# researchmm/MM-Diffusion

Hardware: AMD Instinct MI355X
Metric: denoising steps/sec (video+audio pair), 16x64x64 / 25600 (higher is better)
Workload: dtype bf16; 1 GPU; BASELINE configs[1]: Landscape base model (133.68M params), DDPM p_sample, timestep_respacing=250, per-GPU batch 4, 16x3x64x64 video + 1x25600 audio; global_batch=4, parallelism=batch-sharded x1, no in-loop collective, weights=key-seeded synthetic (mm_diffusion.synth), graph_replay=True, batch_lanes=2, finite=True, ranks_seen=1

## Files before the change

### mm-diffusion_amd/build.py

```python
#!/usr/bin/env python3
import os
import subprocess
import sys

HERE = os.path.dirname(os.path.abspath(__file__))
SRC = os.path.join(HERE, "csrc")
OUT = os.path.join(HERE, "lib", "libmmd.so")
SOURCES = ["mmd_core.hip", "mmd_gemm.hip", "mmd_vconv.hip", "mmd_tattn.hip", "mmd_tconv.hip", "mmd_aconv.hip", "mmd_norm.hip", "mmd_attn.hip", "mmd_misc.hip", "mmd_bwd.hip", "mmd_attn_bwd.hip", "mmd_attn_bwd_mfma.hip"]
FLAGS = ["--offload-arch=gfx950", "-O3", "-std=c++17", "-fPIC", "-ffp-contract=fast", "-Wno-unused-result", "-Wno-inline-asm"]
FLAGS += os.environ.get("MMD_EXTRA_CXXFLAGS", "").split()
NO_PACKED_F32 = ["-Xclang", "-target-feature", "-Xclang", "-packed-fp32-ops"]
FLAGS += NO_PACKED_F32


def _stale():
    if not os.path.exists(OUT):
        return True
    t = os.path.getmtime(OUT)
    deps = [os.path.join(SRC, f) for f in os.listdir(SRC)] + [os.path.abspath(__file__)]
    return any(os.path.getmtime(d) > t for d in deps)


def _llvm_bin():
    cands = [os.environ.get("LLVM_BIN")]
    hipcc = os.environ.get("HIPCC", "/opt/rocm/bin/hipcc")
    try:
        out = subprocess.run([hipcc, "--print-prog-name=llvm-objdump"], stdout=subprocess.PIPE, stderr=subprocess.DEVNULL, timeout=60).stdout.decode().strip()
        if out and os.path.isabs(out):
            cands.append(os.path.dirname(out))
    except (OSError, subprocess.SubprocessError):
        pass
    cands += [os.path.join(os.path.dirname(os.path.dirname(os.path.realpath(hipcc))), "lib", "llvm", "bin"), "/opt/rocm/lib/llvm/bin"]
    for d in cands:
        if d and os.path.exists(os.path.join(d, "llvm-objdump")):
            return d
    raise RuntimeError("build check: llvm-objdump not found (looked in %s); set LLVM_BIN to the LLVM bin directory of the ROCm toolchain"
                       % ", ".join(str(d) for d in cands if d))


def _check_no_packed_f32(path):
    import re
    import tempfile
    llvm = _llvm_bin()
    with tempfile.TemporaryDirectory() as td:
        lib = os.path.join(td, "lib.so")
        os.symlink(os.path.abspath(path), lib)
        subprocess.check_call([os.path.join(llvm, "llvm-objdump"), "--offloading", lib], cwd=td, stdout=subprocess.DEVNULL, stderr=subprocess.DEVNULL)
        cos = sorted(f for f in os.listdir(td) if f.endswith("gfx950"))
        if len(cos) < len(SOURCES) - 1:
            raise RuntimeError("build check: expected >= %d gfx950 code objects in %s, found %d" % (len(SOURCES) - 1, path, len(cos)))
        asm = ""
        for f in cos:
            asm += subprocess.run([os.path.join(llvm, "llvm-objdump"), "-d", "--mcpu=gfx950", os.path.join(td, f)],
                                  stdout=subprocess.PIPE, stderr=subprocess.DEVNULL, check=True).stdout.decode(errors="replace")
    n_mfma = len(re.findall(r"\bv_mfma_", asm))
    bad = re.findall(r"\bv_pk_(?:add|mul|fma)_f32\b", asm)
    if n_mfma == 0:
        raise RuntimeError("build check: the disassembly of %s shows no v_mfma instruction - the check looked at the wrong object" % path)
    if bad:
        raise RuntimeError("build check: %d packed-fp32 instruction(s) (%s ...) in %s: the device pass ignored %s" %
                           (len(bad), bad[0], path, " ".join(NO_PACKED_F32)))


def _check_strip_asm(obj):
    import importlib.util
    spec = importlib.util.spec_from_file_location("strip_asm_check", os.path.join(os.path.dirname(HERE), "tools", "strip_asm_check.py"))
    chk = importlib.util.module_from_spec(spec)
    spec.loader.exec_module(chk)
    chk.LLVM = _llvm_bin()
    n, bad = chk.check(chk.disassemble(obj))
    if n == 0 or bad:
        raise RuntimeError("build check: conv1x1_strip_res_kernel: %d kernels checked, %d violations%s" % (n, len(bad), (": " + bad[0]) if bad else ""))


def build(force=False, verbose=True):
    if not force and not _stale():
        return OUT
    os.makedirs(os.path.dirname(OUT), exist_ok=True)
    hipcc = os.environ.get("HIPCC", "/opt/rocm/bin/hipcc")
    objs = []
    procs = []
    for s in SOURCES:
        o = os.path.join(HERE, "lib", s.replace(".hip", ".o"))
        objs.append(o)
        cmd = [hipcc, *FLAGS, "-c", os.path.join(SRC, s), "-o", o]
        procs.append((cmd, subprocess.Popen(cmd, stdout=subprocess.PIPE, stderr=subprocess.STDOUT)))
    for cmd, p in procs:
        out, _ = p.communicate()
        if p.returncode != 0:
            raise RuntimeError("hipcc failed: %s\n%s" % (" ".join(cmd), out.decode()))
        lines = out.decode().splitlines()
        text = "\n".join(ln for ln in lines if "'-packed-fp32-ops' is not a recognized feature" not in ln).strip()
        if verbose and text:
            print(text)
    tmp = OUT + ".tmp"
    cmd = [hipcc, "--offload-arch=gfx950", "-shared", "-fPIC", "-o", tmp, *objs]
    try:
        subprocess.check_call(cmd)
        _check_no_packed_f32(tmp)
        _check_strip_asm(os.path.join(HERE, "lib", "mmd_gemm.o"))
        os.replace(tmp, OUT)
    finally:
        if os.path.exists(tmp):
            os.remove(tmp)
    if verbose:
        print("built", OUT)
    return OUT


if __name__ == "__main__":
    build(force="--force" in sys.argv)
```

### mm-diffusion_amd/csrc/mmd_common.h

```cpp
#pragma once
#include <hip/hip_runtime.h>
#include <stdint.h>
#include <stdio.h>
#include <stdarg.h>
#include "../../include/mmd.h"

#define MMD_F32 0
#define MMD_BF16 1

#define MMD_OK 0
#define MMD_ERR_ARG (-1)
#define MMD_ERR_LAUNCH (-2)
#define MMD_ERR_UNSUPPORTED (-3)

typedef __attribute__((ext_vector_type(8))) __bf16 bf16x8;
typedef __attribute__((ext_vector_type(4))) __bf16 bf16x4;
typedef __attribute__((ext_vector_type(16))) float f32x16;
typedef __attribute__((ext_vector_type(4))) float f32x4;
typedef __attribute__((ext_vector_type(4))) uint32_t u32x4;
typedef __attribute__((ext_vector_type(2))) uint32_t u32x2;

int mmd_set_error(int code, const char* fmt, ...);
int mmd_check_launch(const char* what);

#define MMD_REQUIRE(cond, ...)                                  \
  do {                                                          \
    if (!(cond)) return mmd_set_error(MMD_ERR_ARG, __VA_ARGS__); \
  } while (0)

__device__ __forceinline__ float bf16_bits_to_f32(uint32_t bits16) { return __uint_as_float(bits16 << 16); }
__device__ __forceinline__ uint32_t f32_to_bf16_bits(float f) {
  uint32_t u = __float_as_uint(f);
  if ((u & 0x7fffffffu) > 0x7f800000u) return 0x7fc0u;
  u += 0x7fffu + ((u >> 16) & 1u);
  return u >> 16;
}
__device__ __forceinline__ uint32_t pack_bf16x2(float lo, float hi) {
  return f32_to_bf16_bits(lo) | (f32_to_bf16_bits(hi) << 16);
}

template <typename T> struct Elt;
template <> struct Elt<float> {
  static constexpr int EPV = 4;
  static constexpr int DT = MMD_F32;
  __device__ static __forceinline__ void unpack(const u32x4& v, float* f) {
#pragma unroll
    for (int i = 0; i < 4; ++i) f[i] = __uint_as_float(v[i]);
  }
  __device__ static __forceinline__ u32x4 pack(const float* f) {
    u32x4 v;
#pragma unroll
    for (int i = 0; i < 4; ++i) v[i] = __float_as_uint(f[i]);
    return v;
  }
  __device__ static __forceinline__ float ld(const void* p, int64_t i) { return ((const float*)p)[i]; }
  __device__ static __forceinline__ void st(void* p, int64_t i, float v) { ((float*)p)[i] = v; }
};
template <> struct Elt<__bf16> {
  static constexpr int EPV = 8;
  static constexpr int DT = MMD_BF16;
  __device__ static __forceinline__ void unpack(const u32x4& v, float* f) {
#pragma unroll
    for (int i = 0; i < 4; ++i) {
      f[2 * i] = __uint_as_float(v[i] << 16);
      f[2 * i + 1] = __uint_as_float(v[i] & 0xffff0000u);
    }
  }
  __device__ static __forceinline__ u32x4 pack(const float* f) {
    bf16x8 t;
#pragma unroll
    for (int i = 0; i < 8; ++i) t[i] = (__bf16)f[i];
    return __builtin_bit_cast(u32x4, t);
  }
  __device__ static __forceinline__ float ld(const void* p, int64_t i) {
    return bf16_bits_to_f32(((const uint16_t*)p)[i]);
  }
  __device__ static __forceinline__ void st(void* p, int64_t i, float v) {
    ((__bf16*)p)[i] = (__bf16)v;
  }
};

__device__ __forceinline__ float silu_f(float x) { return x * __builtin_amdgcn_rcpf(1.0f + __expf(-x)); }

__device__ __forceinline__ float wave_sum(float v) {
#pragma unroll
  for (int o = 32; o > 0; o >>= 1) v += __shfl_xor(v, o, 64);
  return v;
}
__device__ __forceinline__ double wave_sum_d(double v) {
#pragma unroll
  for (int o = 32; o > 0; o >>= 1) v += __shfl_xor(v, o, 64);
  return v;
}
__device__ __forceinline__ float wave_max(float v) {
#pragma unroll
  for (int o = 32; o > 0; o >>= 1) v = fmaxf(v, __shfl_xor(v, o, 64));
  return v;
}

template <int CTRL, int ROWS>
__device__ __forceinline__ float dpp_add(float v) {
  return v + __builtin_bit_cast(float, __builtin_amdgcn_update_dpp(0, __builtin_bit_cast(int, v), CTRL, ROWS, 0xf, false));
}
__device__ __forceinline__ float halfwave_total(float v) {
  v = dpp_add<0x128, 0xf>(v);
  v = dpp_add<0x124, 0xf>(v);
  v = dpp_add<0x122, 0xf>(v);
  v = dpp_add<0x121, 0xf>(v);
  return dpp_add<0x142, 0xa>(v);
}


static inline int cdiv(int64_t a, int64_t b) { return (int)((a + b - 1) / b); }

#define MMD_MAX_DEVICES 16
static inline int mmd_device_slot() {
  int d = 0;
  (void)hipGetDevice(&d);
  return d & (MMD_MAX_DEVICES - 1);
}
```

### mm-diffusion_amd/csrc/mmd_gemm.hip

```cpp
#include "mmd_common.h"

struct ConvGemmParams {
  const char* A; int64_t lda;
  const char* W;
  const float* bias;
  const char* R; int64_t ldr;
  char* Y; int64_t ldy;
  int M, Cout, Cin, ntaps;
  int D0, D1, D2;
  const float* gn_a; const float* gn_b;
  int gn_act, gn_S;
  int64_t gn_rows;
  float* stats; int64_t stats_ld;
  int taps[27 * 3];
};

template <int BM, int BN>
__device__ __forceinline__ void epilogue_stats(const ConvGemmParams& p, float (&sum)[BM / 64][8], float (&sq)[BM / 64][8], float* sP, int m0,
                                               int n0, int tid) {
  constexpr int CVN = BN / 8, NREC = BM / 64;
  const int lane = tid & 63, wave = tid >> 6, cg = tid % CVN;
#pragma unroll
  for (int r = 0; r < NREC; ++r)
#pragma unroll
// ... 1744 lines not shown
  bool& attr_set = attr_done[mmd_device_slot()];
  if (!attr_set) {
    hipError_t e = hipFuncSetAttribute((const void*)conv_gemm_halo_kernel<T, GN>, hipFuncAttributeMaxDynamicSharedMemorySize, (int)lds);
    if (e != hipSuccess) return mmd_set_error(MMD_ERR_LAUNCH, "conv_gemm_halo: set LDS attr: %s", hipGetErrorString(e));
    attr_set = true;
  }
  const int grid = (p.M / 128) * cdiv(p.Cout, 128);
  hipLaunchKernelGGL((conv_gemm_halo_kernel<T, GN>), dim3(grid), dim3(256), lds, st, p);
  return mmd_check_launch("conv_gemm_halo");
}

template <bool GN>
static int launch_conv_gemm_halo16(const ConvGemmParams& p, hipStream_t st) {
  bool taps_ok = p.ntaps == 9;
  for (int t = 0; t < p.ntaps && taps_ok; ++t)
    taps_ok = p.taps[t * 3] == 0 && p.taps[t * 3 + 1] == t / 3 - 1 && p.taps[t * 3 + 2] == t % 3 - 1;
  if (!taps_ok || p.D1 % 16 != 0 || p.D2 % 16 != 0 || (int64_t)p.D0 * p.D1 * p.D2 != p.M || p.Cin % 64 != 0 ||
      ((int64_t)p.D1 * p.D2 - 1) * p.lda * 2 + (int64_t)p.Cin * 2 >= 0x7fffffffLL || (int64_t)128 * p.Cin * 9 * 2 >= 0x7fffffffLL)
    return mmd_set_error(MMD_ERR_UNSUPPORTED, "conv_gemm tile 133 (halo, 16 x 16 patches): needs the nine spatial taps in row-major (dh, dw) order, "
                         "D1 %% 16 == 0, D2 %% 16 == 0, full frames, Cin %% 64 == 0 and frames below 2 GB");
  if (GN && p.gn_rows % ((int64_t)p.D1 * p.D2) != 0)
    return mmd_set_error(MMD_ERR_UNSUPPORTED, "conv_gemm tile 133 with fused GroupNorm: needs slices of whole frames");
  constexpr size_t OPS_B = 2 * (size_t)(41 * 8 * 128) + 3 * (size_t)(128 * 128), C_B = 256 * 132 * sizeof(float);
  const size_t lds = (OPS_B > C_B ? OPS_B : C_B) + 1024 + 256;
  static bool attr_done[MMD_MAX_DEVICES] = {};
  bool& attr_set = attr_done[mmd_device_slot()];
  if (!attr_set) {
    hipError_t e = hipFuncSetAttribute((const void*)conv_gemm_halo16_kernel<GN>, hipFuncAttributeMaxDynamicSharedMemorySize, (int)lds);
    if (e != hipSuccess) return mmd_set_error(MMD_ERR_LAUNCH, "conv_gemm_halo16: set LDS attr: %s", hipGetErrorString(e));
    attr_set = true;
  }
  const int grid = (p.M / 256) * cdiv(p.Cout, 128);
  hipLaunchKernelGGL((conv_gemm_halo16_kernel<GN>), dim3(grid), dim3(512), lds, st, p);
  return mmd_check_launch("conv_gemm_halo16");
}

template <typename T>
static bool glds_desc_ok(const ConvGemmParams& p) {
  static const bool on = [] { const char* e = getenv("MMD_GEMM_DESC"); return !(e && e[0] == '0'); }();
  constexpr int ES = 16 / Elt<T>::EPV;
  int maxshift = 0;
  for (int t = 0; t < p.ntaps; ++t) {
    const int64_t sh = ((int64_t)p.taps[3 * t] * p.D1 * p.D2 + (int64_t)p.taps[3 * t + 1] * p.D2 + p.taps[3 * t + 2]) * p.lda * ES;
    if (sh > 0x3fffffff || sh < -0x3fffffff) return false;
    (void)maxshift;
  }
  return on && ((int64_t)p.M * p.lda + p.Cin) * ES < 0x7fffffffLL && (int64_t)128 * p.Cin * p.ntaps * ES < 0x7fffffffLL;
}

template <typename T>
static int launch_conv_gemm_glds(const ConvGemmParams& p, hipStream_t st) {
  const size_t lds = 128 * 132 * sizeof(float) + 336;
  static bool attr_done[MMD_MAX_DEVICES] = {};
  bool& attr_set = attr_done[mmd_device_slot()];
  if (!attr_set) {
    hipError_t e = hipFuncSetAttribute((const void*)conv_gemm_glds_kernel<T, false, 2, false>, hipFuncAttributeMaxDynamicSharedMemorySize, (int)lds);
    if (e == hipSuccess) e = hipFuncSetAttribute((const void*)conv_gemm_glds_kernel<T, true, 2, false>, hipFuncAttributeMaxDynamicSharedMemorySize, (int)lds);
    if (e == hipSuccess) e = hipFuncSetAttribute((const void*)conv_gemm_glds_kernel<T, true, 2, true>, hipFuncAttributeMaxDynamicSharedMemorySize, (int)lds);
    if (e != hipSuccess) return mmd_set_error(MMD_ERR_LAUNCH, "conv_gemm_glds: set LDS attr: %s", hipGetErrorString(e));
    attr_set = true;
  }
  const int grid = cdiv(p.M, 128) * cdiv(p.Cout, 128);
  if (p.Cin % (8 * Elt<T>::EPV) != 0) hipLaunchKernelGGL((conv_gemm_glds_kernel<T, false, 2, false>), dim3(grid), dim3(256), lds, st, p);
  else if (glds_desc_ok<T>(p)) hipLaunchKernelGGL((conv_gemm_glds_kernel<T, true, 2, true>), dim3(grid), dim3(256), lds, st, p);
  else hipLaunchKernelGGL((conv_gemm_glds_kernel<T, true, 2, false>), dim3(grid), dim3(256), lds, st, p);
  return mmd_check_launch("conv_gemm_glds");
}

template <typename T>
static int launch_conv_gemm_ring(const ConvGemmParams& p, hipStream_t st) {
  if (p.Cin % (8 * Elt<T>::EPV) != 0)
    return mmd_set_error(MMD_ERR_UNSUPPORTED, "conv_gemm tile 132 (deep ring): Cin must be a multiple of one 128-byte K step");
  const size_t lds = 8 * (size_t)(128 * 128) + 336;
  static bool attr_done[MMD_MAX_DEVICES] = {};
  bool& attr_set = attr_done[mmd_device_slot()];
  if (!attr_set) {
    hipError_t e = hipFuncSetAttribute((const void*)conv_gemm_glds_kernel<T, true, 4, false>, hipFuncAttributeMaxDynamicSharedMemorySize, (int)lds);
    if (e == hipSuccess) e = hipFuncSetAttribute((const void*)conv_gemm_glds_kernel<T, true, 4, true>, hipFuncAttributeMaxDynamicSharedMemorySize, (int)lds);
    if (e != hipSuccess) return mmd_set_error(MMD_ERR_LAUNCH, "conv_gemm_ring: set LDS attr: %s", hipGetErrorString(e));
    attr_set = true;
  }
  const int grid = cdiv(p.M, 128) * cdiv(p.Cout, 128);
  if (glds_desc_ok<T>(p)) hipLaunchKernelGGL((conv_gemm_glds_kernel<T, true, 4, true>), dim3(grid), dim3(256), lds, st, p);
  else hipLaunchKernelGGL((conv_gemm_glds_kernel<T, true, 4, false>), dim3(grid), dim3(256), lds, st, p);
  return mmd_check_launch("conv_gemm_ring");
}

template <typename T, int BM, int BN, bool GN>
static int launch_conv_gemm(const ConvGemmParams& p, hipStream_t st) {
  const size_t lds_ops = 2 * (size_t)(BM + BN) * ROWB;
  const size_t lds_c = (size_t)BM * (BN + 4) * sizeof(float);
  const size_t lds = (lds_ops > lds_c ? lds_ops : lds_c) + 336 + (GN ? 16 * 256 : 0);
  static bool attr_done[MMD_MAX_DEVICES] = {};
  bool& attr_set = attr_done[mmd_device_slot()];
  if (!attr_set) {
    hipError_t e = hipFuncSetAttribute((const void*)conv_gemm_kernel<T, BM, BN, GN>,
                                       hipFuncAttributeMaxDynamicSharedMemorySize, (int)lds);
    if (e != hipSuccess) return mmd_set_error(MMD_ERR_LAUNCH, "conv_gemm: set LDS attr: %s", hipGetErrorString(e));
    attr_set = true;
  }
  const int grid = cdiv(p.M, BM) * cdiv(p.Cout, BN);
  hipLaunchKernelGGL((conv_gemm_kernel<T, BM, BN, GN>), dim3(grid), dim3(256), lds, st, p);
  return mmd_check_launch("conv_gemm");
}

template <typename T>
static int dispatch_conv_gemm(const ConvGemmParams& p, int tile, hipStream_t st) {
  if (tile == 133) {
    if constexpr (Elt<T>::EPV == 8) return p.gn_a ? launch_conv_gemm_halo16<true>(p, st) : launch_conv_gemm_halo16<false>(p, st);
    else return mmd_set_error(MMD_ERR_UNSUPPORTED, "conv_gemm tile 133: bf16 only");
  }
  if (p.gn_a) {
    if (tile == 130) {
      if constexpr (Elt<T>::EPV == 8) return launch_conv_gemm_halo<T, true>(p, st);
      else return mmd_set_error(MMD_ERR_UNSUPPORTED, "conv_gemm tile 130 with fused GroupNorm: bf16 only");
    }
    if (tile == 128) return launch_conv_gemm<T, 128, 128, true>(p, st);
    return launch_conv_gemm<T, 64, 64, true>(p, st);
  }
  if (tile == 129) return launch_conv_gemm_glds<T>(p, st);
  if (tile == 132) return launch_conv_gemm_ring<T>(p, st);
  if (tile == 130) return launch_conv_gemm_halo<T, false>(p, st);
  if (tile == 128) return launch_conv_gemm<T, 128, 128, false>(p, st);
  return launch_conv_gemm<T, 64, 64, false>(p, st);
}

static int conv_gemm_impl(int dtype, const void* A, int64_t lda, const void* W, const float* bias, const void* R, int64_t ldr,
                          void* Y, int64_t ldy, int M, int Cout, int Cin, int ntaps, const int* taps, int D0, int D1, int D2,
                          int tile, const float* gn_a, const float* gn_b, int gn_act, int gn_S, int64_t gn_rows, float* stats,
                          int64_t stats_ld, void* stream) {
  const int epv = dtype == MMD_BF16 ? 8 : 4;
  MMD_REQUIRE(dtype == MMD_BF16 || dtype == MMD_F32, "conv_gemm: bad dtype %d", dtype);
  MMD_REQUIRE(A && W && Y && M > 0 && Cout > 0 && Cin > 0, "conv_gemm: null/empty argument");
  MMD_REQUIRE(ntaps >= 1 && ntaps <= 27 && taps, "conv_gemm: ntaps %d out of [1,27]", ntaps);
  MMD_REQUIRE(Cin % epv == 0, "conv_gemm: Cin %d must be a multiple of %d", Cin, epv);
  MMD_REQUIRE(Cout % 8 == 0, "conv_gemm: Cout %d must be a multiple of 8", Cout);
  MMD_REQUIRE(lda % epv == 0 && ldy % epv == 0 && (!R || ldr % epv == 0), "conv_gemm: row strides must be 16-byte multiples");
  MMD_REQUIRE(((uintptr_t)A | (uintptr_t)W | (uintptr_t)Y | (uintptr_t)R) % 16 == 0, "conv_gemm: pointers must be 16-byte aligned");
  MMD_REQUIRE(D0 > 0 && D1 > 0 && D2 > 0, "conv_gemm: bad position dims");
  MMD_REQUIRE(!gn_a || (gn_b && (ntaps == 1 || tile == 130 || tile == 133) && gn_S > 0 && gn_rows >= 128 && (Cin <= 256 || tile == 131 || tile == 130 || tile == 133) &&
                        (int64_t)gn_S * gn_rows == M),
              "gn_conv1x1 / gn_conv_gemm: needs contiguous slices of >= 128 rows covering M, Cin <= 256 unless tile 130 / 131, taps only with tile 130 "
              "(got S=%d rows=%ld Cin=%d M=%d ntaps=%d tile=%d)", gn_S, (long)gn_rows, Cin, M, ntaps, tile);
  ConvGemmParams p;
  p.A = (const char*)A; p.lda = lda; p.W = (const char*)W; p.bias = bias;
  p.R = (const char*)R; p.ldr = ldr; p.Y = (char*)Y; p.ldy = ldy;
  p.M = M; p.Cout = Cout; p.Cin = Cin; p.ntaps = ntaps; p.D0 = D0; p.D1 = D1; p.D2 = D2;
  p.gn_a = gn_a; p.gn_b = gn_b; p.gn_act = gn_act; p.gn_S = gn_S; p.gn_rows = gn_rows;
  MMD_REQUIRE(!stats || (M % 64 == 0 && Cout % 4 == 0 && stats_ld >= Cout / 4 && tile != 130 && tile != 133 && (uintptr_t)stats % 8 == 0),
              "conv_gemm: output statistics need M %% 64 == 0, Cout %% 4 == 0, stats_ld >= Cout / 4 (quads) and a row-tiled main loop (not tiles 130 / 133)");
  p.stats = stats; p.stats_ld = stats_ld;
  for (int i = 0; i < ntaps * 3; ++i) p.taps[i] = taps[i];
  hipStream_t st = (hipStream_t)stream;
  if (tile == 0) tile = (int64_t)cdiv(M, 128) * cdiv(Cout, 128) >= 320 ? 128 : 64;
  MMD_REQUIRE(tile == 64 || tile == 128 || ((tile == 129 || tile == 132) && !gn_a) || (tile == 130 && (!gn_a || dtype == MMD_BF16)) ||
                  ((tile == 131 || tile == 133) && dtype == MMD_BF16),
              "conv_gemm: tile must be 0, 64, 128, 129 (128 direct-to-LDS), 130 (halo-tile 3x3), 131 (row strip, bf16 1x1 convs) or 132 (129 with a "
              "four-slot ring for launches of few tiles)");
  if (tile == 131) return dispatch_conv1x1_strip(p, st);
  return dtype == MMD_BF16 ? dispatch_conv_gemm<__bf16>(p, tile, st) : dispatch_conv_gemm<float>(p, tile, st);
}

extern "C" int mmd_conv_gemm(int dtype, const void* A, int64_t lda, const void* W, const float* bias, const void* R, int64_t ldr,
                             void* Y, int64_t ldy, int M, int Cout, int Cin, int ntaps, const int* taps, int D0, int D1, int D2,
                             int tile, void* stream) {
  return conv_gemm_impl(dtype, A, lda, W, bias, R, ldr, Y, ldy, M, Cout, Cin, ntaps, taps, D0, D1, D2, tile, nullptr, nullptr, 0, 0,
                        0, nullptr, 0, stream);
}

extern "C" int mmd_conv_gemm_stats(int dtype, const void* A, int64_t lda, const void* W, const float* bias, const void* R, int64_t ldr,
                                   void* Y, int64_t ldy, int M, int Cout, int Cin, int ntaps, const int* taps, int D0, int D1, int D2,
                                   int tile, float* stats, int64_t stats_ld, void* stream) {
  MMD_REQUIRE(stats, "conv_gemm_stats: null statistics buffer");
  return conv_gemm_impl(dtype, A, lda, W, bias, R, ldr, Y, ldy, M, Cout, Cin, ntaps, taps, D0, D1, D2, tile, nullptr, nullptr, 0, 0,
                        0, stats, stats_ld, stream);
}

extern "C" int mmd_gn_conv1x1(int dtype, const void* A, int64_t lda, const float* gn_a, const float* gn_b, int act, int S,
                              int64_t rows_per_slice, const void* W, const float* bias, const void* R, int64_t ldr, void* Y,
                              int64_t ldy, int M, int Cout, int Cin, int tile, void* stream) {
  static const int tap0[3] = {0, 0, 0};
  MMD_REQUIRE(gn_a && gn_b, "gn_conv1x1: null GroupNorm affine");
  return conv_gemm_impl(dtype, A, lda, W, bias, R, ldr, Y, ldy, M, Cout, Cin, 1, tap0, 1, 1, 1, tile, gn_a, gn_b, act, S,
                        rows_per_slice, nullptr, 0, stream);
}

extern "C" int mmd_gn_conv1x1_stats(int dtype, const void* A, int64_t lda, const float* gn_a, const float* gn_b, int act, int S,
                                    int64_t rows_per_slice, const void* W, const float* bias, const void* R, int64_t ldr, void* Y,
                                    int64_t ldy, int M, int Cout, int Cin, int tile, float* stats, int64_t stats_ld, void* stream) {
  static const int tap0[3] = {0, 0, 0};
  MMD_REQUIRE(gn_a && gn_b && stats, "gn_conv1x1_stats: null GroupNorm affine / statistics buffer");
  return conv_gemm_impl(dtype, A, lda, W, bias, R, ldr, Y, ldy, M, Cout, Cin, 1, tap0, 1, 1, 1, tile, gn_a, gn_b, act, S,
                        rows_per_slice, stats, stats_ld, stream);
}

extern "C" int mmd_gn_conv_gemm(int dtype, const void* A, int64_t lda, const float* gn_a, const float* gn_b, int act, int S,
                                int64_t rows_per_slice, const void* W, const float* bias, const void* R, int64_t ldr, void* Y,
                                int64_t ldy, int M, int Cout, int Cin, int ntaps, const int* taps, int D0, int D1, int D2, int tile,
                                void* stream) {
  MMD_REQUIRE(gn_a && gn_b, "gn_conv_gemm: null GroupNorm affine");
  MMD_REQUIRE(tile == 130 || tile == 133, "gn_conv_gemm: the fused input GroupNorm of a conv with taps exists on the halo tiles (130 / 133) only");
  return conv_gemm_impl(dtype, A, lda, W, bias, R, ldr, Y, ldy, M, Cout, Cin, ntaps, taps, D0, D1, D2, tile, gn_a, gn_b, act, S,
                        rows_per_slice, nullptr, 0, stream);
}
```

### mm-diffusion_amd/mm_diffusion/ops.py

```python
import math
import os

import torch

from . import _hip as H

GN_EPS = 1e-5

_recorder = None
_keep = None


class recording:
    def __init__(self, plan, keep=None):
        self.plan, self.keep = plan, keep

    def __enter__(self):
        global _recorder, _keep
        self._prev, _recorder = (_recorder, _keep), self.plan
        _keep = self.keep
        return self.plan

    def __exit__(self, *a):
        global _recorder, _keep
# ... 165 lines not shown
        b = alloc(geom.S, C, dtype=torch.float32, device=x.device)
    if out is not None:
        _chk2d(out)
    _dispatch("mmd_gn_group", H.dt_of(x), x.data_ptr(), x.stride(0), H.ptr(out), 0 if out is None else out.stride(0), C, *geom.args(),
              gamma.data_ptr(), beta.data_ptr(), H.ptr(film), 0 if film is None else film.stride(0), GN_EPS, 1 if act else 0,
              H.ptr(a), H.ptr(b), H.ptr(mr),
              meta=(f"gn_group[S={geom.S},Tn={geom.Tn},C={C}]", 0, (1 if out is None else 2) * geom.S * geom.Tn * C * x.element_size()))
    return (a, b) if out is None else out


def add_rowbias(x, e, rows_per_sample):
    _chk2d(x)
    _dispatch("mmd_add_rowbias", H.dt_of(x), x.data_ptr(), x.stride(0), x.shape[0], x.shape[1], rows_per_sample,
           e.data_ptr(), e.stride(0))
    return x


def colsum_slices(dy, out, rows_per_sample):
    _chk2d(dy)
    S = dy.shape[0] // rows_per_sample
    _dispatch("mmd_colsum_slices", H.dt_of(dy), dy.data_ptr(), dy.stride(0), S, rows_per_sample, dy.shape[1], out.data_ptr(), out.stride(0))
    return out


TAPS_1 = [(0, 0, 0)]
TAPS_SPATIAL = [(0, dh, dw) for dh in (-1, 0, 1) for dw in (-1, 0, 1)]
TAPS_TEMPORAL = [(df, 0, 0) for df in (-1, 0, 1)]
TAPS_TEMPORAL_D1 = [(0, df, 0) for df in (-1, 0, 1)]
TAPS_3D = [(df, dh, dw) for df in (-1, 0, 1) for dh in (-1, 0, 1) for dw in (-1, 0, 1)]


def taps_audio(dilation):
    return [(-dilation, 0, 0), (0, 0, 0), (dilation, 0, 0)]


AUTOTUNE = True
_tile_cache = {}


def _pick_tile(key, launch, M, Cout, candidates=(64, 128, 129), out=None, scratch=()):
    default = (129 if 129 in candidates else 128) if ((M + 127) // 128) * ((Cout + 127) // 128) >= 320 else 64
    if default not in candidates:
        default = candidates[0]
    if not AUTOTUNE or _recorder is None:
        return default
    key = (key, tuple(candidates))
    if key in _tile_cache:
        return _tile_cache[key]
    import ctypes
    verify = out is not None and not any(t is not None and t.untyped_storage().data_ptr() == out.untyped_storage().data_ptr() for t in scratch)
    saved = []
    if verify:
        for t in scratch:
            if t is not None:
                saved.append((t, t.clone()))
                t.normal_()
    best, best_ms, ref = default, None, None
    ev = [ctypes.c_void_p(), ctypes.c_void_p()]
    for e in ev:
        H.call("mmd_event_create", ctypes.byref(e))
    st = H.stream_handle()
    for tile in candidates:
        launch(tile)
        if verify:
            if ref is None:
                ref = out.clone()
            elif tile == 130:
                err = float((out.float() - ref.float()).norm() / ref.float().norm().clamp_min(1e-30))
                if not err < (1e-2 if out.element_size() == 2 else 1e-5):
                    raise H.MMDError(f"conv_gemm tile 130 disagrees with tile {candidates[0]} on {key}: rel-L2 {err:.3e}")
            elif not torch.equal(out.view(torch.int16 if out.element_size() == 2 else torch.int32),
                                 ref.view(torch.int16 if ref.element_size() == 2 else torch.int32)):
                raise H.MMDError(f"GEMM tile {tile} is not bitwise equal to tile {candidates[0]} on {key}")
        t_min = None
        for _ in range(2):
            H.call("mmd_event_record", ev[0], st)
            for _ in range(5):
                launch(tile)
            H.call("mmd_event_record", ev[1], st)
            ms = ctypes.c_float()
            H.call("mmd_event_elapsed_ms", ev[0], ev[1], ctypes.byref(ms))
            t_min = ms.value if t_min is None else min(t_min, ms.value)
        if best_ms is None or t_min < best_ms:
            best, best_ms = tile, t_min
    for e in ev:
        H.lib().mmd_event_destroy(e)
    for t, keep in saved:
        t.copy_(keep)
    _tile_cache[key] = best
    return best


_HALO_MODE = os.environ.get("MMD_GEMM_HALO", "pin")
HALO_CANDIDATE = _HALO_MODE == "1"


def halo_tile_ok(x, taps, dims):
    M, Cin = x.shape
    return (len(taps) > 1 and all(t[0] == 0 and abs(t[1]) <= 1 and abs(t[2]) <= 1 for t in taps) and dims[1] % 8 == 0
            and dims[2] % 16 == 0 and dims[0] * dims[1] * dims[2] == M and Cin % (128 // x.element_size()) == 0)


_HALO16 = os.environ.get("MMD_HALO16", "1") != "0"


def halo_tile_code(x, taps, dims):
    return 133 if (_HALO16 and x.dtype == torch.bfloat16 and len(taps) == 9 and dims[1] % 16 == 0 and dims[2] % 16 == 0
                   and x.shape[1] >= 256 and tuple(tuple(t) for t in taps) == tuple(TAPS_SPATIAL)) else 130


def _stats_args(stats, M, Cout):
    if (stats.dtype != torch.float32 or Cout % 4 or tuple(stats.shape) != (M // 64, Cout // 4, 2) or M % 64 or stats.stride(1) != 2
            or stats.stride(2) != 1):
        raise H.MMDError(f"GEMM output statistics: expected an fp32 [M/64, Cout/4, 2] view, got {tuple(stats.shape)} strides {stats.stride()}")
    return stats.data_ptr(), stats.stride(0) // 2


_HALO_MIN_PIXELS = int(os.environ.get("MMD_HALO_MIN_PIXELS", "1024"))


def halo_tile_pinned(x, taps, dims):
    return (_HALO_MODE == "pin" and x.dtype == torch.bfloat16 and len(taps) == 9 and dims[1] * dims[2] >= _HALO_MIN_PIXELS
            and halo_tile_ok(x, taps, dims))


_STRIP_MODE = os.environ.get("MMD_GEMM_STRIP", "pin")


def strip_tile_ok(x, Cout, taps=TAPS_1, stats=None, geom=None, base=False):
    M, Cin = x.shape
    K = len(taps) * Cin
    if x.dtype != torch.bfloat16 or K not in (128, 256, 384, 512) or Cin % 64:
        return False
    if len(taps) == 1 and tuple(taps[0]) != (0, 0, 0):
        return False
    rf = 2 if K <= 256 else 1
    if Cout % (32 * rf) or Cout > 2048 or (stats is not None and M % 64):
        return False
    if base and (len(taps) != 1 or K == 512 or (stats is not None and rf != 2)):
        return False
    if geom is not None and not (len(taps) == 1 and geom.inner == 1 and geom.tstride == 1 and geom.outer_stride == geom.Tn
                                 and geom.Tn >= 128 * rf and geom.S * geom.Tn == M):
        return False
    return True


def strip_tile_pinned(x, Cout, taps=TAPS_1, stats=None, geom=None):
    if _STRIP_MODE == "0":
        return False
    return strip_tile_ok(x, Cout, taps, stats, geom, base=_STRIP_MODE == "base")


def _tile_name(tile):
    return {129: "128glds", 130: "128halo", 131: "strip", 132: "128ring", 133: "256halo"}.get(tile, tile)


_RING_MODE = os.environ.get("MMD_GEMM_RING", "1")


def ring_tile_candidate(x, Cout, ntaps):
    M, Cin = x.shape
    kstep = 128 // x.element_size()
    return (_RING_MODE != "0" and Cin % kstep == 0 and (Cin * ntaps) // kstep >= 4
            and ((M + 127) // 128) * ((Cout + 127) // 128) <= 384)


def conv_gemm(x, w, bias, taps=TAPS_1, dims=(1, 1, 1), residual=None, out=None, tile=0, stats=None):
    _chk2d(x)
    M, Cin = x.shape
    Cout = w.shape[0]
    if w.dtype != x.dtype or w.shape[1] != len(taps) * Cin or not w.is_contiguous():
        raise H.MMDError(f"conv_gemm: weight {tuple(w.shape)} {w.dtype} does not match input {tuple(x.shape)} {x.dtype} x {len(taps)} taps")
    out = alloc(M, Cout, dtype=x.dtype, device=x.device) if out is None else out
    _chk2d(out)
    arr, nt = H.taps_array(taps)
    es = x.element_size()
    base = (H.dt_of(x), x.data_ptr(), x.stride(0), w.data_ptr(), H.ptr(bias), H.ptr(residual),
            0 if residual is None else residual.stride(0), out.data_ptr(), out.stride(0), M, Cout, Cin, nt, arr,
            int(dims[0]), int(dims[1]), int(dims[2]))
    if tile == 0 and stats is None and halo_tile_pinned(x, taps, dims):
        tile = halo_tile_code(x, taps, dims)
    if tile == 0 and strip_tile_pinned(x, Cout, taps, stats):
        tile = 131
    if tile == 0:
        cands = (128, 129) if stats is not None else (64, 128, 129) + ((130,) if HALO_CANDIDATE and halo_tile_ok(x, taps, dims) else ())
        if ring_tile_candidate(x, Cout, nt):
            cands = cands + (132,)
        tile = _pick_tile((es, M, Cin, nt, Cout, residual is not None, False, tuple(dims) if 130 in cands else None),
                          lambda t: H.call("mmd_conv_gemm", *base, t, H.stream_handle()), M, Cout, cands, out=out, scratch=(x, residual))
    flops = 2 * M * Cout * Cin * nt
    nbytes = es * (M * Cin + M * Cout * (2 if residual is not None else 1) + Cout * Cin * nt) + 4 * Cout
    label = f"conv_gemm<{'bf16' if es == 2 else 'f32'},{_tile_name(tile)}>[M={M},K={Cin * nt},N={Cout}]"
    if stats is not None:
        _dispatch("mmd_conv_gemm_stats", *base, tile, *_stats_args(stats, M, Cout), meta=(label, flops, nbytes))
    else:
        _dispatch("mmd_conv_gemm", *base, tile, meta=(label, flops, nbytes))
    return out


_STRIP_BLOCKS_RULE = int(os.environ.get("MMD_STRIP_BLOCKS_RULE", "448"))


def strip_column_split(M, K, Cout):
    rf, cc = (2, 64) if K <= 256 else (1, 32)
    rowblocks, nch, n = -(-M // (128 * rf)), Cout // cc, 1
    for d in range(1, min(nch, 16) + 1):
        if nch % d == 0:
            n = d
            if rowblocks * d >= _STRIP_BLOCKS_RULE:
                break
    return n


def gn_fusable(geom: Geom, Cin, Cout, x=None, stats=None, act=False):
    if x is not None and strip_tile_pinned(x, Cout, stats=stats):
        if not strip_tile_pinned(x, Cout, stats=stats, geom=geom):
            return False
        return not (act and strip_column_split(x.shape[0], Cin, Cout) > 2)
    return (geom.inner == 1 and geom.tstride == 1 and geom.outer_stride == geom.Tn and geom.Tn >= 128 and Cin <= 256
            and (Cout + 127) // 128 <= 2)


def gn_conv1x1(x, a, b, geom: Geom, act, w, bias, residual=None, out=None, tile=0, stats=None):
    _chk2d(x)
    M, Cin = x.shape
    Cout = w.shape[0]
    if w.dtype != x.dtype or w.shape[1] != Cin or not w.is_contiguous():
        raise H.MMDError(f"gn_conv1x1: weight {tuple(w.shape)} {w.dtype} does not match input {tuple(x.shape)} {x.dtype}")
    out = alloc(M, Cout, dtype=x.dtype, device=x.device) if out is None else out
    _chk2d(out)
    es = x.element_size()
    tiled_ok = (geom.inner == 1 and geom.tstride == 1 and geom.outer_stride == geom.Tn and geom.Tn >= 128 and Cin <= 256
                and (Cout + 127) // 128 <= 2)
    strip_ok = strip_tile_ok(x, Cout, stats=stats, geom=geom)
    if not ((tile == 131 and strip_ok) or (tile in (64, 128) and tiled_ok) or (tile == 0 and (tiled_ok or strip_ok))):
        raise H.MMDError("gn_conv1x1: needs contiguous slices of >= 128 rows, Cin <= 256 (use gn_apply + conv_gemm otherwise)")
    base = (H.dt_of(x), x.data_ptr(), x.stride(0), a.data_ptr(), b.data_ptr(), 1 if act else 0, geom.S, geom.Tn,
            w.data_ptr(), H.ptr(bias), H.ptr(residual),
            0 if residual is None else residual.stride(0), out.data_ptr(), out.stride(0), M, Cout, Cin)
    if tile == 0 and strip_tile_pinned(x, Cout, stats=stats, geom=geom):
        tile = 131
    if tile == 0 and not tiled_ok:
        raise H.MMDError("gn_conv1x1: the row-strip kernel is switched off (MMD_GEMM_STRIP) and the tiled loader cannot take this launch")
    if tile == 0:
        tile = _pick_tile((es, M, Cin, 1, Cout, residual is not None, True),
                          lambda t: H.call("mmd_gn_conv1x1", *base, t, H.stream_handle()), M, Cout,
                          candidates=(128,) if stats is not None else (64, 128), out=out, scratch=(x, residual, a, b))
    nbytes = es * (M * Cin + M * Cout * (2 if residual is not None else 1) + Cout * Cin) + 4 * Cout
    meta = (f"gn_conv1x1<{'bf16' if es == 2 else 'f32'},{_tile_name(tile)}>[M={M},K={Cin},N={Cout}]", 2 * M * Cout * Cin, nbytes)
    if stats is not None:
        _dispatch("mmd_gn_conv1x1_stats", *base, tile, *_stats_args(stats, M, Cout), meta=meta)
    else:
        _dispatch("mmd_gn_conv1x1", *base, tile, meta=meta)
    return out


_HALO_GN = os.environ.get("MMD_HALO_GN", "1") != "0"


def halo_gn_ok(x, taps, dims, geom: Geom):
    return (_HALO_GN and halo_tile_pinned(x, taps, dims) and geom.inner == 1 and geom.tstride == 1 and geom.outer_stride == geom.Tn
            and geom.S * geom.Tn == x.shape[0] and geom.Tn % (dims[1] * dims[2]) == 0)


def gn_conv_gemm(x, a, b, geom: Geom, act, w, bias, taps, dims, residual=None, out=None, tile=0):
    _chk2d(x)
    M, Cin = x.shape
    Cout = w.shape[0]
    if w.dtype != x.dtype or w.shape[1] != len(taps) * Cin or not w.is_contiguous():
        raise H.MMDError(f"gn_conv_gemm: weight {tuple(w.shape)} {w.dtype} does not match input {tuple(x.shape)} {x.dtype} x {len(taps)} taps")
    if not (halo_tile_ok(x, taps, dims) and len(taps) == 9 and x.dtype == torch.bfloat16 and geom.S * geom.Tn == M
            and geom.inner == 1 and geom.tstride == 1 and geom.outer_stride == geom.Tn and geom.Tn % (dims[1] * dims[2]) == 0):
        raise H.MMDError("gn_conv_gemm: needs a bf16 3x3 conv tile 130 accepts and contiguous slices of whole frames")
    out = alloc(M, Cout, dtype=x.dtype, device=x.device) if out is None else out
    _chk2d(out)
    arr, nt = H.taps_array(taps)
    es = x.element_size()
    flops = 2 * M * Cout * Cin * nt
    nbytes = es * (M * Cin + M * Cout * (2 if residual is not None else 1) + Cout * Cin * nt) + 4 * Cout
    _dispatch("mmd_gn_conv_gemm", H.dt_of(x), x.data_ptr(), x.stride(0), a.data_ptr(), b.data_ptr(), 1 if act else 0, geom.S, geom.Tn,
              w.data_ptr(), H.ptr(bias), H.ptr(residual), 0 if residual is None else residual.stride(0), out.data_ptr(), out.stride(0),
              M, Cout, Cin, nt, arr, int(dims[0]), int(dims[1]), int(dims[2]), tile or halo_tile_code(x, taps, dims),
              meta=(f"gn_conv_gemm<bf16,{_tile_name(tile or halo_tile_code(x, taps, dims))}>[M={M},K={Cin * nt},N={Cout}]", flops, nbytes))
    return out


_VCONV_FUSED = os.environ.get("MMD_VCONV_FUSED", "1") != "0"


def vconv_shape_ok(x, Cout, N, F, Hh, Ww):
    return (x.dtype == torch.bfloat16 and F == 16 and Cout == 128 and x.shape[1] % 32 == 0 and Hh % 4 == 0 and Ww % 4 == 0
            and x.shape[0] == N * F * Hh * Ww and (16 * Hh * Ww * x.stride(0) + x.shape[1]) * 2 < 2 ** 31)


def _ranges_overlap(x, y):
    x0, y0 = x.data_ptr(), y.data_ptr()
    x1 = x0 + ((x.shape[0] - 1) * x.stride(0) + x.shape[1]) * x.element_size()
    y1 = y0 + ((y.shape[0] - 1) * y.stride(0) + y.shape[1]) * y.element_size()
    return not (x1 <= y0 or y1 <= x0)


def vconv_fused_ok(x, Cout, N, F, Hh, Ww, out=None):
    return _VCONV_FUSED and vconv_shape_ok(x, Cout, N, F, Hh, Ww) and (out is None or not _ranges_overlap(x, out))


def vconv_pack(ws, wt):
    H.require_cuda(ws, wt)
    Cout, Cin = ws.shape[0], ws.shape[1] // 9
    if ws.dtype != torch.bfloat16 or wt.dtype != torch.bfloat16 or tuple(wt.shape) != (Cout, 3 * Cout) or not ws.is_contiguous() or not wt.is_contiguous():
        raise H.MMDError(f"vconv_pack: expected contiguous bf16 [Cout, 9 Cin] / [Cout, 3 Cout], got {tuple(ws.shape)} / {tuple(wt.shape)}")
    out = torch.empty(H.lib().mmd_vconv2d1d_weight_bytes(Cin) // 2, dtype=torch.bfloat16, device=ws.device)
    H.call("mmd_vconv2d1d_pack", ws.data_ptr(), wt.data_ptr(), out.data_ptr(), Cin, Cout, H.stream_handle())
    return out


def vconv2d1d(x, wf, bias_s, bias_t, N, F, Hh, Ww, a=None, b=None, geom=None, act=True, out=None, stats=None):
    _chk2d(x)
    M, Cin = x.shape
    Cout = 128
    if not vconv_shape_ok(x, Cout, N, F, Hh, Ww):
        raise H.MMDError(f"vconv2d1d: unsupported launch (x {tuple(x.shape)} {x.dtype}, N={N} F={F} H={Hh} W={Ww})")
    if (a is None) != (b is None) or (a is not None and (geom is None or geom.inner != 1 or geom.tstride != 1 or geom.outer_stride != geom.Tn
                                                         or geom.S * geom.Tn != M or geom.Tn % (F * Hh * Ww))):
        raise H.MMDError("vconv2d1d: the fused input norm needs contiguous slices of whole samples")
    out = alloc(M, Cout, dtype=x.dtype, device=x.device) if out is None else out
    _chk2d(out)
    if _ranges_overlap(x, out) or tuple(out.shape) != (M, Cout) or out.dtype != x.dtype:
        raise H.MMDError("vconv2d1d: the output must be a bf16 [M, 128] tensor whose address range does not overlap the input's (the C side "
                         "compares whole ranges: column slices of one buffer count as overlapping)")
    if wf.numel() * wf.element_size() != H.lib().mmd_vconv2d1d_weight_bytes(Cin):
        raise H.MMDError("vconv2d1d: the weight image does not match Cin (pack it with vconv_pack)")
    sp, sld = (None, 0) if stats is None else _stats_args(stats, M, Cout)
    flops = 2 * M * Cout * (9 * Cin + 3 * Cout)
    nbytes = 2 * (M * Cin + M * Cout + Cout * (9 * Cin + 3 * Cout)) + 8 * Cout
    _dispatch("mmd_vconv2d1d", x.data_ptr(), x.stride(0), H.ptr(a), H.ptr(b), 1 if act else 0, 0 if geom is None else geom.S,
              0 if geom is None else geom.Tn, wf.data_ptr(), H.ptr(bias_s), H.ptr(bias_t), out.data_ptr(), out.stride(0), N, F, Hh, Ww, Cin, Cout,
              sp, sld, meta=(f"vconv2d1d<bf16{',gn' if a is not None else ''}>[M={M},Cin={Cin},N={Cout}]", flops, nbytes))
    return out


# ... 471 lines not shown
```

Baseline: 364.6 pair-steps/s.

## Add frame-resident 3x3 conv GEMM tile for 8x8 frames as autotune candidate

```diff
diff --git a/mm-diffusion_amd/build.py b/mm-diffusion_amd/build.py
--- a/mm-diffusion_amd/build.py
+++ b/mm-diffusion_amd/build.py
@@ -6,7 +6,7 @@
 HERE = os.path.dirname(os.path.abspath(__file__))
 SRC = os.path.join(HERE, "csrc")
 OUT = os.path.join(HERE, "lib", "libmmd.so")
-SOURCES = ["mmd_core.hip", "mmd_gemm.hip", "mmd_vconv.hip", "mmd_tattn.hip", "mmd_tconv.hip", "mmd_aconv.hip", "mmd_norm.hip", "mmd_attn.hip", "mmd_misc.hip", "mmd_bwd.hip", "mmd_attn_bwd.hip", "mmd_attn_bwd_mfma.hip"]
+SOURCES = ["mmd_core.hip", "mmd_gemm.hip", "mmd_fconv.hip", "mmd_vconv.hip", "mmd_tattn.hip", "mmd_tconv.hip", "mmd_aconv.hip", "mmd_norm.hip", "mmd_attn.hip", "mmd_misc.hip", "mmd_bwd.hip", "mmd_attn_bwd.hip", "mmd_attn_bwd_mfma.hip"]
 FLAGS = ["--offload-arch=gfx950", "-O3", "-std=c++17", "-fPIC", "-ffp-contract=fast", "-Wno-unused-result", "-Wno-inline-asm"]
 FLAGS += os.environ.get("MMD_EXTRA_CXXFLAGS", "").split()
 NO_PACKED_F32 = ["-Xclang", "-target-feature", "-Xclang", "-packed-fp32-ops"]
diff --git a/mm-diffusion_amd/csrc/mmd_common.h b/mm-diffusion_amd/csrc/mmd_common.h
--- a/mm-diffusion_amd/csrc/mmd_common.h
+++ b/mm-diffusion_amd/csrc/mmd_common.h
@@ -22,6 +22,9 @@
 
 int mmd_set_error(int code, const char* fmt, ...);
 int mmd_check_launch(const char* what);
+int mmd_fconv_dispatch(int dtype, const void* A, int64_t lda, const void* W, const float* bias, const void* R, int64_t ldr, void* Y,
+                       int64_t ldy, int M, int Cout, int Cin, int ntaps, const int* taps, int D0, int D1, int D2, bool extras,
+                       hipStream_t st);
 
 #define MMD_REQUIRE(cond, ...)                                  \
   do {                                                          \
diff --git a/mm-diffusion_amd/csrc/mmd_fconv.hip b/mm-diffusion_amd/csrc/mmd_fconv.hip
--- /dev/null
+++ b/mm-diffusion_amd/csrc/mmd_fconv.hip
@@ -0,0 +1,271 @@
+#include "mmd_common.h"
+
+struct FConvParams {
+  const char* A; int64_t lda;
+  const char* W;
+  const float* bias;
+  const char* R; int64_t ldr;
+  char* Y; int64_t ldy;
+  int M, Cout, Cin;
+};
+
+#define FCONV_FENCE() __builtin_amdgcn_sched_barrier(0)
+#define FCONV_LAUNDER4(v) asm volatile("" : "+v"((v).x), "+v"((v).y), "+v"((v).z), "+v"((v).w))
+
+__device__ __attribute__((aligned(16))) uint32_t g_fconv_zero[4] = {0, 0, 0, 0};
+
+__device__ __forceinline__ void fconv_wait_vm(int n) {
+  if (n >= 8) {
+    if (n >= 28) asm volatile("s_waitcnt vmcnt(28)" ::: "memory");
+    else if (n >= 24) asm volatile("s_waitcnt vmcnt(24)" ::: "memory");
+    else if (n >= 20) asm volatile("s_waitcnt vmcnt(20)" ::: "memory");
+    else if (n >= 16) asm volatile("s_waitcnt vmcnt(16)" ::: "memory");
+    else if (n >= 12) asm volatile("s_waitcnt vmcnt(12)" ::: "memory");
+    else if (n >= 10) asm volatile("s_waitcnt vmcnt(10)" ::: "memory");
+    else asm volatile("s_waitcnt vmcnt(8)" ::: "memory");
+  } else if (n >= 4) {
+    if (n >= 6) asm volatile("s_waitcnt vmcnt(6)" ::: "memory");
+    else if (n == 5) asm volatile("s_waitcnt vmcnt(5)" ::: "memory");
+    else asm volatile("s_waitcnt vmcnt(4)" ::: "memory");
+  } else {
+    if (n == 3) asm volatile("s_waitcnt vmcnt(3)" ::: "memory");
+    else if (n == 2) asm volatile("s_waitcnt vmcnt(2)" ::: "memory");
+    else if (n == 1) asm volatile("s_waitcnt vmcnt(1)" ::: "memory");
+    else asm volatile("s_waitcnt vmcnt(0)" ::: "memory");
+  }
+}
+
+template <int FR, int BN, int NS>
+__global__ __launch_bounds__(256, 1) void fconv_kernel(const FConvParams p) {
+#if defined(__HIP_DEVICE_COMPILE__)
+  constexpr int BM = FR * 64;
+  constexpr int SLAB = (BM + 2) * 128;
+  constexpr int WST = BN * 128;
+  constexpr int RT = BM / 32;
+  constexpr int TN = (RT * (BN / 32)) / 4;
+  constexpr int AI = BM / 32;
+  constexpr int NW = BN / 32;
+  constexpr int LDC = BN + 4;
+  constexpr int STEADY = (NS - 2) * NW;
+  static_assert(RT * (BN / 32) >= 4 && NS >= 3, "four waves, each at least one 32 x 32 tile");
+  extern __shared__ __attribute__((aligned(16))) char smem[];
+  const int NSL = p.Cin >> 6;
+  char* sA = smem;
+  char* sW = smem + NSL * SLAB;
+  float* sC = (float*)smem;
+
+  const int tid = threadIdx.x;
+  const int lane = tid & 63;
+  const int wave = __builtin_amdgcn_readfirstlane(tid >> 6);
+  const int half = lane >> 5, l31 = lane & 31;
+  const int rt = wave % RT, ct0 = (wave / RT) * TN;
+
+  const int Mt = (p.M + BM - 1) / BM;
+  int wgid;
+  {
+    const int nwg = gridDim.x, bid = blockIdx.x, q = nwg >> 3, r = nwg & 7, xcd = bid & 7;
+    wgid = (xcd < r ? xcd * (q + 1) : r * (q + 1) + (xcd - r) * q) + (bid >> 3);
+  }
+  const int nt = wgid / Mt, mt = wgid - nt * Mt;
+  const int m0 = mt * BM, n0 = nt * BN;
+  const int K2 = p.Cin * 9 * 2;
+  const int nit = NSL * 9;
+
+  typedef __attribute__((address_space(3))) void* lptr_t;
+  const uint32_t OOB = 0xfffffff0u;
+  const auto rsrcA = __builtin_amdgcn_make_buffer_rsrc((void*)p.A, 0, (int)(((int64_t)p.M - 1) * p.lda * 2 + (int64_t)p.Cin * 2), 0x00020000);
+  const auto rsrcW = __builtin_amdgcn_make_buffer_rsrc((void*)(p.W + (int64_t)n0 * K2), 0, BN * K2, 0x00020000);
+  const int lrow = lane >> 3, pc = lane & 7;
+  uint32_t a_voff[AI], w_voff[NW];
+#pragma unroll
+  for (int i = 0; i < AI; ++i) {
+    const int row = (wave * AI + i) * 8 + lrow;
+    const int m = m0 + row;
+    a_voff[i] = m < p.M ? (uint32_t)((int64_t)m * p.lda * 2 + ((pc ^ ((row >> 1) & 7)) << 4)) : OOB;
+  }
+#pragma unroll
+  for (int i = 0; i < NW; ++i) {
+    const int row = (wave * NW + i) * 8 + lrow;
+    w_voff[i] = (uint32_t)(row * K2 + ((pc ^ ((row >> 1) & 7)) << 4));
+  }
+  auto issue_w = [&](int k, int slot) {
+#pragma unroll
+    for (int i = 0; i < NW; ++i)
+      __builtin_amdgcn_raw_ptr_buffer_load_lds(rsrcW, (lptr_t)(sW + slot * WST + (wave * NW + i) * 1024), 16, w_voff[i], k * 128, 0, 0);
+  };
+
+  constexpr int CVN = BN / 8, RP = 256 / CVN, NPASS = BM / RP;
+  const int e_cg = tid % CVN, e_rr = tid / CVN;
+  const int e_co = n0 + e_cg * 8;
+  float bs[8];
+#pragma unroll
+  for (int j = 0; j < 8; ++j) bs[j] = p.bias ? p.bias[e_co + j] : 0.f;
+
+  for (int k = 0; k < NS; ++k) issue_w(k, k);
+  for (int s = 0; s < NSL; ++s) {
+#pragma unroll
+    for (int i = 0; i < AI; ++i)
+      __builtin_amdgcn_raw_ptr_buffer_load_lds(rsrcA, (lptr_t)(sA + s * SLAB + (wave * AI + i) * 1024), 16, a_voff[i], s * 128, 0, 0);
+  }
+  for (int t = tid; t < NSL * 16; t += 256) *(u32x4*)(sA + (t >> 4) * SLAB + BM * 128 + (t & 15) * 16) = u32x4{0, 0, 0, 0};
+  int iss = NS * NW + NSL * AI;
+  auto allowed = [&](int j) {
+    const int pw = j < NS ? (j + 1) * NW : NS * NW + NSL * AI + (j - NS + 1) * NW;
+    const int pa = j < NSL ? NS * NW + (j + 1) * AI : 0;
+    return iss - (pw > pa ? pw : pa);
+  };
+
+  f32x16 acc[TN];
+#pragma unroll
+  for (int a = 0; a < TN; ++a)
+#pragma unroll
+    for (int r = 0; r < 16; ++r) acc[a][r] = 0.f;
+
+  const int xsw = (l31 >> 1) & 7;
+  uint32_t w_foff[4], a_foff[4];
+#pragma unroll
+  for (int c = 0; c < 4; ++c) w_foff[c] = (uint32_t)((ct0 * 32 + l31) * 128 + (((2 * c + half) ^ xsw) << 4));
+  const int arow = rt * 32 + l31, py = (arow >> 3) & 7, px = arow & 7;
+  int r_tap = 0, r_s = 0;
+  struct Frag { u32x4 w[4][TN]; u32x4 a[4]; };
+  auto read = [&](Frag& f, int slot) {
+    if (r_s == 0) {
+      const int dh = r_tap / 3 - 1, dw = r_tap - (r_tap / 3) * 3 - 1;
+      const bool ok = (unsigned)(py + dh) < 8u && (unsigned)(px + dw) < 8u;
+      const int rs = arow + dh * 8 + dw;
+#pragma unroll
+      for (int c = 0; c < 4; ++c)
+        a_foff[c] = (uint32_t)((ok ? rs : BM + (rs & 1)) * 128 + (((2 * c + half) ^ ((rs >> 1) & 7)) << 4));
+    }
+    const char* bW = sW + slot * WST;
+    const char* bA = sA + r_s * SLAB;
+#pragma unroll
+    for (int c = 0; c < 4; ++c) {
+#pragma unroll
+      for (int a = 0; a < TN; ++a) f.w[c][a] = *(const u32x4*)(bW + a * 32 * 128 + w_foff[c]);
+      f.a[c] = *(const u32x4*)(bA + a_foff[c]);
+    }
+    if (++r_s == NSL) { r_s = 0; ++r_tap; }
+  };
+  auto mm = [&](const Frag& f) {
+#pragma unroll
+    for (int c = 0; c < 4; ++c)
+#pragma unroll
+      for (int a = 0; a < TN; ++a)
+        acc[a] = __builtin_amdgcn_mfma_f32_32x32x16_bf16(__builtin_bit_cast(bf16x8, f.w[c][a]), __builtin_bit_cast(bf16x8, f.a[c]), acc[a], 0, 0, 0);
+  };
+
+  Frag f0, f1;
+  int slot_r = 0;
+  fconv_wait_vm(allowed(0));
+  __syncthreads();
+  read(f0, 0);
+  slot_r = 1;
+  auto step = [&](int it, const Frag& cur, Frag& nxt) {
+    const int n = allowed(it + 1);
+    if (n == STEADY) asm volatile("s_waitcnt vmcnt(%0)" ::"n"(STEADY) : "memory");
+    else fconv_wait_vm(n);
+    asm volatile("s_waitcnt lgkmcnt(0)" ::: "memory");
+    __builtin_amdgcn_s_barrier();
+    asm volatile("" ::: "memory");
+    if (it + NS < nit) {
+      int slot_w = slot_r - 1;
+      if (slot_w < 0) slot_w += NS;
+      issue_w(it + NS, slot_w);
+      iss += NW;
+    }
+    read(nxt, slot_r);
+    if (++slot_r == NS) slot_r = 0;
+    FCONV_FENCE();
+    mm(cur);
+    FCONV_FENCE();
+  };
+  for (int it = 0; it + 2 < nit; it += 2) {
+    step(it, f0, f1);
+    step(it + 1, f1, f0);
+  }
+  step(nit - 2, f0, f1);
+  u32x4 rres[NPASS];
+  if (p.R) {
+#pragma unroll
+    for (int ps = 0; ps < NPASS; ++ps) {
+      const int m = m0 + e_rr + ps * RP;
+      rres[ps] = *(const u32x4*)(m < p.M ? p.R + ((int64_t)m * p.ldr + e_co) * 2 : (const char*)g_fconv_zero);
+    }
+  }
+  mm(f1);
+  __syncthreads();
+  if (p.R) {
+#pragma unroll
+    for (int ps = 0; ps < NPASS; ++ps) FCONV_LAUNDER4(rres[ps]);
+  }
+
+#pragma unroll
+  for (int a = 0; a < TN; ++a) {
+    const int ml = rt * 32 + l31;
+#pragma unroll
+    for (int q = 0; q < 4; ++q) {
+      const int col = (ct0 + a) * 32 + 8 * q + 4 * half;
+      f32x4 v = {acc[a][4 * q], acc[a][4 * q + 1], acc[a][4 * q + 2], acc[a][4 * q + 3]};
+      *(f32x4*)(sC + ml * LDC + col) = v;
+    }
+  }
+  __syncthreads();
+#pragma unroll
+  for (int ps = 0; ps < NPASS; ++ps) {
+    const int ml = e_rr + ps * RP;
+    const int m = m0 + ml;
+    if (m < p.M) {
+      float v[8];
+      const f32x4 c0 = *(const f32x4*)(sC + ml * LDC + e_cg * 8);
+      const f32x4 c1 = *(const f32x4*)(sC + ml * LDC + e_cg * 8 + 4);
+#pragma unroll
+      for (int j = 0; j < 4; ++j) { v[j] = c0[j] + bs[j]; v[4 + j] = c1[j] + bs[4 + j]; }
+      if (p.R) {
+        float rf[8];
+        Elt<__bf16>::unpack(rres[ps], rf);
+#pragma unroll
+        for (int j = 0; j < 8; ++j) v[j] += rf[j];
+      }
+      *(u32x4*)(p.Y + ((int64_t)m * p.ldy + e_co) * 2) = Elt<__bf16>::pack(v);
+    }
+  }
+#endif
+}
+
+template <int FR, int BN, int NS>
+static int launch_fconv(const FConvParams& p, hipStream_t st) {
+  constexpr int BM = FR * 64;
+  const size_t lds = (size_t)(p.Cin / 64) * (BM + 2) * 128 + (size_t)NS * BN * 128;
+  static bool attr_done = false;
+  if (!attr_done) {
+    hipError_t e = hipFuncSetAttribute((const void*)fconv_kernel<FR, BN, NS>, hipFuncAttributeMaxDynamicSharedMemorySize, 160 * 1024);
+    if (e != hipSuccess) return mmd_set_error(MMD_ERR_LAUNCH, "conv_gemm tile 138: set LDS attr: %s", hipGetErrorString(e));
+    attr_done = true;
+  }
+  const int grid = ((p.M + BM - 1) / BM) * (p.Cout / BN);
+  hipLaunchKernelGGL((fconv_kernel<FR, BN, NS>), dim3(grid), dim3(256), lds, st, p);
+  return mmd_check_launch("conv_gemm_fconv");
+}
+
+int mmd_fconv_dispatch(int dtype, const void* A, int64_t lda, const void* W, const float* bias, const void* R, int64_t ldr, void* Y,
+                       int64_t ldy, int M, int Cout, int Cin, int ntaps, const int* taps, int D0, int D1, int D2, bool extras,
+                       hipStream_t st) {
+  MMD_REQUIRE(dtype == MMD_BF16 && !extras, "conv_gemm tile 138 (frame-resident 3x3): bf16 only, no fused GroupNorm, no output statistics");
+  bool taps_ok = ntaps == 9;
+  for (int t = 0; taps_ok && t < 9; ++t) taps_ok = taps[3 * t] == 0 && taps[3 * t + 1] == t / 3 - 1 && taps[3 * t + 2] == t % 3 - 1;
+  MMD_REQUIRE(taps_ok, "conv_gemm tile 138 (frame-resident 3x3): needs the nine spatial taps (0, dh, dw) in row-major order");
+  MMD_REQUIRE(D1 == 8 && D2 == 8 && (int64_t)D0 * 64 == M, "conv_gemm tile 138 (frame-resident 3x3): needs 8 x 8 frames of contiguous rows, M = D0 * 64 "
+              "(got dims %d x %d x %d, M %d)", D0, D1, D2, M);
+  MMD_REQUIRE(Cin % 128 == 0 && Cin <= 1024 && Cout % 64 == 0, "conv_gemm tile 138 (frame-resident 3x3): needs Cin %% 128 == 0, Cin <= 1024, Cout %% 64 == 0 "
+              "(got Cin %d Cout %d)", Cin, Cout);
+  MMD_REQUIRE(((int64_t)M - 1) * lda * 2 + (int64_t)Cin * 2 < (int64_t)0x7fffffff, "conv_gemm tile 138: the activation view must stay below 2 GB");
+  FConvParams p;
+  p.A = (const char*)A; p.lda = lda; p.W = (const char*)W; p.bias = bias; p.R = (const char*)R; p.ldr = ldr; p.Y = (char*)Y; p.ldy = ldy;
+  p.M = M; p.Cout = Cout; p.Cin = Cin;
+#ifdef FCONV_WIDE
+  if (Cin <= 512) return launch_fconv<2, 64, 3>(p, st);
+#endif
+  if (Cin <= 512) return launch_fconv<2, 32, 6>(p, st);
+  return launch_fconv<1, 64, 3>(p, st);
+}
diff --git a/mm-diffusion_amd/csrc/mmd_gemm.hip b/mm-diffusion_amd/csrc/mmd_gemm.hip
--- a/mm-diffusion_amd/csrc/mmd_gemm.hip
+++ b/mm-diffusion_amd/csrc/mmd_gemm.hip
@@ -1920,11 +1920,13 @@
   p.stats = stats; p.stats_ld = stats_ld;
   for (int i = 0; i < ntaps * 3; ++i) p.taps[i] = taps[i];
   hipStream_t st = (hipStream_t)stream;
+  if (tile == 138)
+    return mmd_fconv_dispatch(dtype, A, lda, W, bias, R, ldr, Y, ldy, M, Cout, Cin, ntaps, taps, D0, D1, D2, gn_a || stats, st);
   if (tile == 0) tile = (int64_t)cdiv(M, 128) * cdiv(Cout, 128) >= 320 ? 128 : 64;
   MMD_REQUIRE(tile == 64 || tile == 128 || ((tile == 129 || tile == 132) && !gn_a) || (tile == 130 && (!gn_a || dtype == MMD_BF16)) ||
                   ((tile == 131 || tile == 133) && dtype == MMD_BF16),
-              "conv_gemm: tile must be 0, 64, 128, 129 (128 direct-to-LDS), 130 (halo-tile 3x3), 131 (row strip, bf16 1x1 convs) or 132 (129 with a "
-              "four-slot ring for launches of few tiles)");
+              "conv_gemm: tile must be 0, 64, 128, 129 (128 direct-to-LDS), 130 (halo-tile 3x3), 131 (row strip, bf16 1x1 convs), 132 (129 with a "
+              "four-slot ring for launches of few tiles) or 138 (frame-resident 3x3 on 8 x 8 frames)");
   if (tile == 131) return dispatch_conv1x1_strip(p, st);
   return dtype == MMD_BF16 ? dispatch_conv_gemm<__bf16>(p, tile, st) : dispatch_conv_gemm<float>(p, tile, st);
 }
diff --git a/mm-diffusion_amd/mm_diffusion/ops.py b/mm-diffusion_amd/mm_diffusion/ops.py
--- a/mm-diffusion_amd/mm_diffusion/ops.py
+++ b/mm-diffusion_amd/mm_diffusion/ops.py
@@ -341,7 +341,7 @@
 
 
 def _tile_name(tile):
-    return {129: "128glds", 130: "128halo", 131: "strip", 132: "128ring", 133: "256halo"}.get(tile, tile)
+    return {129: "128glds", 130: "128halo", 131: "strip", 132: "128ring", 133: "256halo", 138: "frame"}.get(tile, tile)
 
 
 _RING_MODE = os.environ.get("MMD_GEMM_RING", "1")
@@ -352,6 +352,20 @@
     kstep = 128 // x.element_size()
     return (_RING_MODE != "0" and Cin % kstep == 0 and (Cin * ntaps) // kstep >= 4
             and ((M + 127) // 128) * ((Cout + 127) // 128) <= 384)
+
+
+_FCONV_MODE = os.environ.get("MMD_GEMM_FCONV", "1")
+
+
+def fconv_tile_ok(x, Cout, taps, dims):
+    M, Cin = x.shape
+    return (x.dtype == torch.bfloat16 and tuple(tuple(t) for t in taps) == tuple(TAPS_SPATIAL) and int(dims[1]) == 8 and int(dims[2]) == 8
+            and int(dims[0]) * 64 == M and Cin % 128 == 0 and Cin <= 1024 and Cout % 64 == 0
+            and ((M - 1) * x.stride(0) + Cin) * 2 < 2 ** 31 - 1)
+
+
+def fconv_tile_candidate(x, Cout, taps, dims, stats=None):
+    return _FCONV_MODE != "0" and stats is None and fconv_tile_ok(x, Cout, taps, dims)
 
 
 def conv_gemm(x, w, bias, taps=TAPS_1, dims=(1, 1, 1), residual=None, out=None, tile=0, stats=None):
@@ -375,6 +389,8 @@
         cands = (128, 129) if stats is not None else (64, 128, 129) + ((130,) if HALO_CANDIDATE and halo_tile_ok(x, taps, dims) else ())
         if ring_tile_candidate(x, Cout, nt):
             cands = cands + (132,)
+        if fconv_tile_candidate(x, Cout, taps, dims, stats):
+            cands = cands + (138,)
         tile = _pick_tile((es, M, Cin, nt, Cout, residual is not None, False, tuple(dims) if 130 in cands else None),
                           lambda t: H.call("mmd_conv_gemm", *base, t, H.stream_handle()), M, Cout, cands, out=out, scratch=(x, residual))
     flops = 2 * M * Cout * Cin * nt
```

After: 359.1 pair-steps/s, median of 2. -1.5%, worse.
